# whwh747/A-Low-Texture-Robust-Hybrid-Feature-Based-Visual-Odometry

Measured on AMD Instinct MI355X. Metric: RGB-D frames/sec (640×480, 1k ORB + LSD + PEAC) at 1/2/4/8 GPUs, higher is better.
Workload: dtype u8/u16 integer + f32/f64; 1 GPU; 640x480 synthetic RGB-D, 1000 ORB (quota; 3/4 std + 1/4 lowtex scenes) + LSD lines + PEAC planes, 8192 frames per GPU per step (std640); frames_per_gpu=8192, parallelism=frames sharded, 1 rank(s), no data-path collective, distinct_frames=256, resident_bytes_per_frame_estimate=21100000

## Files before the change

a-low-texture-robust-hybrid-feature-based-visual-odometry_amd/csrc/peac.hip:

```cpp
#include <type_traits>
#include "hvo_internal.hpp"
#include <math.h>
#include <stdlib.h>
#include <string.h>
#include <vector>
#include <algorithm>

#define WIN 10
#define MIN_SUPPORT 3000
#define MAX_PLANES 64
#define SEG_D 16
#define SEG_I 8
#define LCAP 1024

struct PeacPlan {
    int w = 0, h = 0, pitch = 0, Nw = 0, Nh = 0, nblk = 0, segcap = 0, poolcap = 0, qcap = 0, batch = 0;
    uint16_t *d_depth = nullptr;
    double *d_segD = nullptr; int *d_segI = nullptr; int *d_pool = nullptr, *d_pool2 = nullptr;
    int *d_parent = nullptr, *d_dsize = nullptr, *d_eflag = nullptr;
    int *d_meta = nullptr;
    int *d_extracted = nullptr;
    int *d_blkmap = nullptr; int8_t *d_labels = nullptr; uint32_t *d_state = nullptr;
    int *d_queue = nullptr; int *d_plidmap = nullptr; int *d_isvalid = nullptr;
    hvo_plane *d_planes = nullptr;
    unsigned long long *d_adj = nullptr;
    void *d_hot = nullptr;
    double *d_hkey = nullptr, *d_m1k = nullptr; int *d_hid = nullptr;
    int *d_lq = nullptr;
    double c15 = 0, c60 = 0, c30 = 0;
    double ang_factor = 0, ang_near = 0;
    struct { Knob edges, gl, perm, lend, slots, heads_maxn, heads, heads_big, poolcap, ldsq, flood_t, flood_epl, flood_perm, flood_delay; } kn;
};

static PeacPlan *plan_of(hvo_ctx *ctx) { return (PeacPlan *)ctx->peac; }

static __device__ __forceinline__ void eig33_smallest_dev(double a, double b, double c, double d, double e, double f, double &l0, double v[3])
{
    const double tol = 2.220446049250313e-16 * (a + b + c);
    double l = 0.0;
    bool go = true;
#pragma unroll 1
    for (int it = 0; it < 8; it++) {
        if (!__any(go)) break;
        const double A = a - l, B = b - l, C = c - l;
        const double m1 = B * C - e * e, m2 = A * C - f * f, m3 = A * B - d * d;
        const double det = A * m1 - d * (d * C - e * f) + f * (d * e - B * f);
        const double dq = m1 + m2 + m3;
        const double q2 = -2.0 * (A + B + C);
        double disc = 4.0 * dq * dq + 6.0 * det * q2;
        if (disc < 0.0) disc = 0.0;
        const double ln = l + 3.0 * det / (dq + sqrt(disc));
        const bool adv = go && (dq > 0.0) && (ln > l);
        const double step = ln - l;
        if (adv) l = ln;
        go = adv && !(step <= tol);
    }
    const double A = a - l, B = b - l, C = c - l;
    const double m1 = B * C - e * e, m2 = A * C - f * f, m3 = A * B - d * d;
    const double am1 = fabs(m1), am2 = fabs(m2), am3 = fabs(m3);
    double x, y, z;
    if (am1 >= am2 && am1 >= am3) { x = m1; y = e * f - d * C; z = d * e - B * f; }
    else if (am2 >= am3) { x = e * f - d * C; y = m2; z = d * f - A * e; }
    else { x = d * e - B * f; y = d * f - A * e; z = m3; }
    const double n2 = x * x + y * y + z * z;
// ... 1154 lines not shown
            }
        }
        blkmap[b] = plid;
    }
    __syncthreads();
    const int tw = FS_TW(w), nrows = tw * FS_TH(h) * 4;
    for (int i = slice * 256 + tid; i < nrows; i += 256 * nslices) {
        const int t = i >> 2, ty = t / tw, tx = t - ty * tw;
        const int x0 = tx * 8, y = ty * 4 + (i & 3);
        if (y >= h) continue;
        const int by = y / WIN, bx0 = x0 / WIN, xs = (bx0 + 1) * WIN;
        const int l0 = (by < Nh && bx0 < Nw) ? blkmap[by * Nw + bx0] : -1, l1 = (by < Nh && bx0 + 1 < Nw) ? blkmap[by * Nw + bx0 + 1] : -1;
        unsigned dd[4];
        if (x0 + 8 <= pitch) { const uint4 q = *reinterpret_cast<const uint4 *>(D + (size_t)y * pitch + x0); dd[0] = q.x; dd[1] = q.y; dd[2] = q.z; dd[3] = q.w; }
        else { for (int k = 0; k < 4; k++) { const int xa = x0 + 2 * k; dd[k] = (xa < w ? (unsigned)D[(size_t)y * pitch + xa] : 0u) | ((xa + 1 < w ? (unsigned)D[(size_t)y * pitch + xa + 1] : 0u) << 16); } }
        unsigned st[8];
#pragma unroll
        for (int k = 0; k < 8; k++) {
            const int lab = x0 + k < xs ? l0 : l1;
            st[k] = FS_MAKE(lab, lab >= 0, (dd[k >> 1] >> (16 * (k & 1))) & 0xFFFFu);
        }
        uint4 *dst = reinterpret_cast<uint4 *>(state + (size_t)i * 8);
        dst[0] = make_uint4(st[0], st[1], st[2], st[3]); dst[1] = make_uint4(st[4], st[5], st[6], st[7]);
    }
}

struct RfArgs {
    ClArgs c;
    const uint16_t *depth; size_t dframe; int pitch, w, h;
    float fx, fy, cx, cy, dfac;
    int *blkmap; int *isvalid; uint32_t *state; int *queue; int qcap; int *plidmap; const int *perm;
    hvo_plane *planes; double c30;
    int flood_delay;
};

#ifndef FLOOD_HS_MUL
#define FLOOD_HS_MUL 1
#endif
#define FQ_PACK(x, y, pl) (((pl) << 26) | ((y) << 13) | (x))
static __device__ __forceinline__ void lds_barrier()
{
    __builtin_amdgcn_fence(__ATOMIC_RELEASE, "workgroup", "local");
    __builtin_amdgcn_s_barrier();
    __builtin_amdgcn_fence(__ATOMIC_ACQUIRE, "workgroup", "local");
}
template <int FLOOD_T, int EPL>
#ifdef HVO_WPE_FLOOD
__attribute__((amdgpu_waves_per_eu(HVO_WPE_FLOOD)))
#endif
__global__ __launch_bounds__(FLOOD_T) void k_peac_flood(RfArgs r, unsigned long long *__restrict__ adj_out)
{
    constexpr int NENT = FLOOD_T * EPL, NEV = NENT * 4;
    constexpr int FLOOD_HS = NEV * FLOOD_HS_MUL, FLOOD_HL = 4, FLOOD_NP = 4 * EPL;
    constexpr int NW = FLOOD_T / 64;
    static_assert(NEV <= 2048, "the group lists hold 11-bit event indices");
    constexpr int IXB = NEV > 1024 ? 11 : 10;
    constexpr unsigned IXM = (1u << IXB) - 1u;
    constexpr bool HL8 = NEV <= 256;
    typedef typename std::conditional<HL8, unsigned char, typename std::conditional<(NEV > 1024), unsigned int, unsigned short>::type>::type hl_t;
    __shared__ double pl[MAX_PLANES][7];
    __shared__ unsigned long long adj[MAX_PLANES], simok[MAX_PLANES];
    __shared__ int hkeys[FLOOD_HS], hcnt[FLOOD_HS];
    __shared__ __attribute__((aligned(16))) hl_t hlist[FLOOD_HS * FLOOD_HL];
    __shared__ uint2 rec[NEV];
    static_assert(FLOOD_HS >= NEV, "a ranked round indexes hkeys / hcnt by compact event index");
    __shared__ int wsum[EPL * NW], psum[FLOOD_NP * NW];
    __shared__ int s_nq, s_cx[2];
    const ClArgs &a = r.c;
    const int frame = r.perm ? r.perm[blockIdx.x] : (int)blockIdx.x, tid = threadIdx.x, lane = tid & 63, wv = tid >> 6;
    const int w = r.w, h = r.h, Nw = a.Nw, nblk = a.nblk;
    int *meta = a.meta + (size_t)frame * 16;
    const int nold = meta[2];
    const int *ext = a.extracted + (size_t)frame * 2 * MAX_PLANES;
    const double *segD = a.segD + (size_t)frame * a.segcap * SEG_D;
    const int *blkmap = r.blkmap + (size_t)frame * nblk;
    uint32_t *state = r.state + (size_t)frame * FS_FRAME(w, h);
    const int stw = FS_TW(w);
    int *queue = r.queue + (size_t)frame * r.qcap;
    int flags = 0;
    if (tid < MAX_PLANES) {
        adj[tid] = 0;
        if (tid < nold) { const double *sd = segD + (size_t)ext[tid] * SEG_D; for (int k = 0; k < 7; k++) pl[tid][k] = sd[9 + k]; }
    }
    for (int i = tid; i < FLOOD_HS; i += FLOOD_T) { hkeys[i] = -1; hcnt[i] = 0; }
    if (tid < 2) s_cx[tid] = 0;
    __syncthreads();
    if (tid < MAX_PLANES) {
        unsigned long long m = 0;
        if (tid < nold) for (int q = 0; q < nold; q++) {
            const double *P = pl[tid], *Q = pl[q];
            if (fabs(P[3] * Q[3] + P[4] * Q[4] + P[5] * Q[5]) >= r.c30) m |= 1ull << q;
        }
        simok[tid] = m;
    }
    constexpr int SEED_MAXG = 256;
    __shared__ int gtot[NW > 1 ? SEED_MAXG : 1];
    auto seed_count = [&](int b, int &m, int &up, int &lf, int &i, int &j) {
        int cnt = 0; m = -2; up = -2; lf = -2; i = 0; j = 0;
        if (b < nblk) {
            i = b / Nw; j = b - i * Nw; m = blkmap[b];
            up = i > 0 ? blkmap[b - Nw] : -2; lf = j > 0 ? blkmap[b - 1] : -2;
            if (m < 0) { if (i > 0 && up >= 0) cnt += WIN - 1; if (j > 0 && lf >= 0) cnt += WIN - 1; }
            else { if (i > 0 && up != m) cnt += WIN - 1; if (j > 0 && lf != m) cnt += WIN - 1; }
        }
        return cnt;
    };
    auto seed_write = [&](int pos, int cnt, int m, int up, int lf, int i, int j) {
        if (cnt && pos + cnt <= r.qcap) {
            const int x0 = j * WIN, y0 = i * WIN;
            if (m < 0) {
                if (i > 0 && up >= 0) for (int k = 1; k < WIN; ++k) queue[pos++] = FQ_PACK(x0 + k, y0 - 1, up);
                if (j > 0 && lf >= 0) for (int k = 0; k < WIN - 1; ++k) queue[pos++] = FQ_PACK(x0 - 1, y0 + k, lf);
            } else {
                if (i > 0 && up != m) for (int k = 0; k < WIN - 1; ++k) queue[pos++] = FQ_PACK(x0 + k, y0, m);
                if (j > 0 && lf != m) for (int k = 1; k < WIN; ++k) queue[pos++] = FQ_PACK(x0, y0 + k, m);
            }
        }
    };
    const int ngrp = (nblk + 63) / 64;
    if (NW > 1 && ngrp <= SEED_MAXG) {
        for (int g = wv; g < ngrp; g += NW) {
            int m, up, lf, i, j;
            int incl = seed_count(g * 64 + lane, m, up, lf, i, j);
            for (int o = 1; o < 64; o <<= 1) { int t = __shfl_up(incl, o); if (lane >= o) incl += t; }
// ... 97 lines not shown
                    if (act) actm |= 1u << (e * 4 + j);
                    const unsigned long long bm = __ballot(act);
                    below[e] += __popcll(bm & ltm); etot[e] += __popcll(bm);
                }
            }
            if (NW > 1) {
                if (lane == 0) for (int e = 0; e < EPL; e++) wsum[e * NW + wv] = etot[e];
                lds_barrier();
#pragma unroll
                for (int e = 0; e < EPL; e++) {
                    off[e] = wtot;
                    for (int i = 0; i < NW; i++) { const int v = wsum[e * NW + i]; if (i < wv) off[e] += v; wtot += v; }
                }
            } else {
#pragma unroll
                for (int e = 0; e < EPL; e++) { off[e] = wtot; wtot += etot[e]; }
            }
#pragma unroll
            for (int e = 0; e < EPL; e++) {
                const int plid = (int)((unsigned)q[e] >> 26), sx = q[e] & 8191, sy = (q[e] >> 13) & 8191;
                const int px[4] = { sx - 1, sx + 1, sx, sx }, py[4] = { sy, sy, sy - 1, sy + 1 };
                int c = off[e] + below[e];
#pragma unroll
                for (int j = 0; j < 4; j++) if (actm & (1u << (e * 4 + j))) { rec[c] = make_uint2((unsigned)FQ_PACK(px[j], py[j], plid), st[e][j]); c++; }
            }
        }
        lds_barrier();
        const int na = __builtin_amdgcn_readfirstlane(wtot);
        const int npass = (na + FLOOD_T - 1) / FLOOD_T;
#ifdef HVO_PEAC_TIMING
        if (tid == 0) { atomicAdd(&g_peac_t[30], (unsigned long long)na); atomicAdd(&g_peac_t[31], (unsigned long long)npass); }
#endif
        FT(1)
        unsigned eq[FLOOD_NP], es[FLOOD_NP]; float ed[FLOOD_NP], ecd[FLOOD_NP]; bool eok[FLOOD_NP], ev[FLOOD_NP], push[FLOOD_NP]; int hs[FLOOD_NP], eix[FLOOD_NP];
#pragma unroll
        for (int p = 0; p < FLOOD_NP; p++) {
            ev[p] = false; push[p] = false; eq[p] = 0; es[p] = 0; ed[p] = 0; ecd[p] = -1; eok[p] = false; hs[p] = 0; eix[p] = 0;
            if (p < npass) {
                const int c = p * FLOOD_T + tid;
                ev[p] = c < na;
                if (ev[p]) {
                    const uint2 R = rec[c];
                    eq[p] = R.x; es[p] = R.y;
                    const int ep = (int)(R.x >> 26), ex_ = (int)(R.x & 8191u), ey = (int)((R.x >> 13) & 8191u);
                    eix[p] = FS_IDX(ex_, ey, stw);
                    geom(pl[ep], ex_, ey, (int)(R.y >> 16), FS_LABEL(R.y), ecd[p], eok[p], ed[p]);
                    int s = (int)(((unsigned)eix[p] * 2654435761u) >> 19) & (FLOOD_HS - 1);
                    for (;;) {
                        const int old = atomicCAS(&hkeys[s], -1, eix[p]);
                        if (old == -1 || old == eix[p]) break;
                        s = (s + 1) & (FLOOD_HS - 1);
                    }
                    const int pos = atomicAdd(&hcnt[s], 1);
                    if (pos < FLOOD_HL) hlist[s * FLOOD_HL + pos] = HL8 ? (hl_t)c : (hl_t)((ep << IXB) | c);
                    hs[p] = s;
                }
            }
        }
        lds_barrier();
        bool first[FLOOD_NP], multi[FLOOD_NP]; int cnt[FLOOD_NP]; int cx = 0;
#pragma unroll
        for (int p = 0; p < FLOOD_NP; p++) {
            first[p] = false; multi[p] = false; cnt[p] = 1;
            if (p < npass && ev[p]) {
                cnt[p] = hcnt[hs[p]];
                first[p] = true;
                if (cnt[p] > FLOOD_HL) cx |= 2;
                else if (cnt[p] > 1) {
                    const unsigned me = ((eq[p] >> 26) << IXB) | (unsigned)(p * FLOOD_T + tid);
                    const hl_t *hp_ = &hlist[hs[p] * FLOOD_HL];
                    unsigned l[4] = { hp_[0], hp_[1], hp_[2], hp_[3] };
                    if (HL8) {
#pragma unroll
                        for (int t = 0; t < 4; t++) if (t < cnt[p]) l[t] |= (rec[l[t]].x >> 26) << IXB;
                    }
#pragma unroll
                    for (int t = 0; t < 4; t++) if (t < cnt[p]) {
                        if ((l[t] ^ me) >> IXB) multi[p] = true;
                        if ((l[t] & IXM) < (me & IXM)) first[p] = false;
                    }
                    if (multi[p]) cx |= FS_LABEL(es[p]) < 0 ? 1 : 2;
                }
            }
        }
        if (cx) atomicOr(&s_cx[par], cx);
        lds_barrier();
        const int cxr = s_cx[par];
        const bool complex_round = (cxr & 2) != 0;
        if (r.flood_delay && (cxr & 1) && wv == 0)
            for (int i = 0; i < r.flood_delay; i++) __builtin_amdgcn_s_sleep(127);
#pragma unroll
        for (int p = 0; p < FLOOD_NP; p++) if (p < npass && ev[p]) { hkeys[hs[p]] = -1; hcnt[hs[p]] = 0; }
        FT(2)
        int total = 0;
        if (!complex_round) {
#pragma unroll
            for (int p = 0; p < FLOOD_NP; p++) {
                if (p < npass && first[p] && !multi[p]) {
                    const int ep = (int)(eq[p] >> 26), trail = FS_LABEL(es[p]);
                    const bool closer = eok[p] && ecd[p] < ed[p];
                    if (eok[p] && trail >= 0 && ((simok[ep] >> trail) & 1ull)) { atomicOr(&adj[trail], 1ull << ep); atomicOr(&adj[ep], 1ull << trail); }
                    const int nl = closer ? ep : (trail < 0 ? max(trail - cnt[p], -6) : trail);
                    push[p] = closer;
                    if (nl != trail) state[eix[p]] = (es[p] & ~0xFFu) | ((unsigned)nl & 0xFFu);
                }
            }
            if (cxr & 1) {
                n_ranked++;
#ifdef HVO_PEAC_TIMING
                ft[6]++;
#endif
                if (NW > 1) lds_barrier();
#pragma unroll
                for (int p = 0; p < FLOOD_NP; p++) if (p < npass && multi[p]) hkeys[p * FLOOD_T + tid] = (int)(eok[p] ? __float_as_uint(ecd[p]) : 0xFFFFFFFFu);
                lds_barrier();
#pragma unroll
                for (int p = 0; p < FLOOD_NP; p++) {
                    if (p < npass && first[p] && multi[p]) {
                        const hl_t *hp_ = &hlist[hs[p] * FLOOD_HL];
                        unsigned l[4] = { hp_[0], hp_[1], hp_[2], hp_[3] };
                        if (HL8) {
#pragma unroll
                            for (int t = 0; t < 4; t++) if (t < cnt[p]) l[t] |= (rec[l[t]].x >> 26) << IXB;
                        }
                        int trail = FS_LABEL(es[p]); float dist = ed[p];
                        int last = -1;
                        for (int it = 0; it < cnt[p]; it++) {
                            unsigned best = 0; int c = 1 << 20;
#pragma unroll
                            for (int t = 0; t < 4; t++) { const int ct = (int)(l[t] & IXM); if (t < cnt[p] && ct > last && ct < c) { c = ct; best = l[t]; } }
                            const int ep = (int)(best >> IXB);
                            last = c;
                            const unsigned okcd = (unsigned)hkeys[c];
                            const bool ok = okcd != 0xFFFFFFFFu; const float cd = __uint_as_float(okcd);
                            const bool live = !(trail <= -6 || trail == ep);
                            const bool closer = live && ok && cd < dist;
                            if (live && ok && trail >= 0 && ((simok[ep] >> trail) & 1ull)) { atomicOr(&adj[trail], 1ull << ep); atomicOr(&adj[ep], 1ull << trail); }
                            trail = closer ? ep : ((live && trail < 0) ? trail - 1 : trail);
                            dist = closer ? cd : dist;
                            hcnt[c] = closer ? 1 : 0;
                        }
                        state[eix[p]] = (es[p] & ~0xFFu) | ((unsigned)trail & 0xFFu);
                    }
                }
                lds_barrier();
#pragma unroll
                for (int p = 0; p < FLOOD_NP; p++) if (p < npass && multi[p]) { push[p] = hcnt[p * FLOOD_T + tid] != 0; hkeys[p * FLOOD_T + tid] = -1; hcnt[p * FLOOD_T + tid] = 0; }
            }
            unsigned long long bm[FLOOD_NP]; int off[FLOOD_NP];
#pragma unroll
            for (int p = 0; p < FLOOD_NP; p++) { bm[p] = 0; if (p < npass) bm[p] = __ballot(push[p]); }
            if (NW > 1) {
                if (lane == 0) for (int p = 0; p < FLOOD_NP; p++) psum[p * NW + wv] = __popcll(bm[p]);
                lds_barrier();
#pragma unroll
                for (int p = 0; p < FLOOD_NP; p++) {
                    off[p] = total;
                    for (int i = 0; i < NW; i++) { const int v = psum[p * NW + i]; if (i < wv) off[p] += v; total += v; }
                }
            } else {
#pragma unroll
                for (int p = 0; p < FLOOD_NP; p++) { off[p] = total; total += __popcll(bm[p]); }
            }
#pragma unroll
            for (int p = 0; p < FLOOD_NP; p++) if (p < npass && push[p]) {
                const int pos = nq + off[p] + __popcll(bm[p] & ltm);
                if (pos < r.qcap) queue[pos] = (int)eq[p];
            }
        } else {
            n_serial++;
#ifdef HVO_PEAC_TIMING
            ft[5]++;
#endif
            if (tid == 0) {
                int nqs = nq;
                for (int e = 0; e < nent; e++) {
                    const int qq = queue[kq + e];
                    const int ep = (int)((unsigned)qq >> 26), x0 = qq & 8191, y0 = (qq >> 13) & 8191;
                    for (int j = 0; j < 4; j++) {
                        const int x = x0 + (j == 0 ? -1 : j == 1 ? 1 : 0), y = y0 + (j == 2 ? -1 : j == 3 ? 1 : 0);
                        if (x < 0 || x >= w || y < 0 || y >= h) continue;
                        const int ix = FS_IDX(x, y, stw);
                        const uint32_t s = state[ix];
                        int trail = FS_LABEL(s); float dist;
                        if ((s & FS_VALID) || trail <= -6 || trail == ep) continue;
                        float cd; bool ok;
                        geom(pl[ep], x, y, (int)(s >> 16), trail, cd, ok, dist);
                        if (ok) {
                            if (trail >= 0 && ((simok[ep] >> trail) & 1ull)) { atomicOr(&adj[trail], 1ull << ep); atomicOr(&adj[ep], 1ull << trail); }
                            if (cd < dist) { trail = ep; dist = cd; if (nqs < r.qcap) queue[nqs] = FQ_PACK(x, y, ep); nqs++; }
                            else if (trail < 0) trail -= 1;
                        } else if (trail < 0) trail -= 1;
                        state[ix] = (s & ~0xFFu) | ((unsigned)trail & 0xFFu);
                    }
                }
                s_nq = nqs - nq;
            }
            lds_barrier();
            total = s_nq;
        }
        nq += total;
        if (nq > r.qcap) { nq = r.qcap; flags |= 32; }
        kq += nent;
        par ^= 1;
        __syncthreads();
        FT(3)
    }
#ifdef HVO_PEAC_TIMING
    if (tid == 0) { for (int q = 0; q < 6; q++) atomicAdd(&g_peac_t[16 + q], ft[q]); for (int q = 6; q < 12; q++) atomicAdd(&g_peac_t[18 + q], ft[q]); atomicAdd(&g_peac_t[22], (unsigned long long)nq); atomicAdd(&g_peac_t[23], 1ull); }
#endif
    if (tid < MAX_PLANES) adj_out[(size_t)frame * MAX_PLANES + tid] = adj[tid];
    if (tid == 0) { meta[5] = nq; meta[7] = flags; meta[8] = n_rounds; meta[9] = n_ranked; meta[10] = n_serial; }
}

__global__ __launch_bounds__(64) void k_peac_final(RfArgs r, const unsigned long long *__restrict__ adj_in)
{
    __shared__ double hkey[MAX_PLANES]; __shared__ int hid[MAX_PLANES];
    __shared__ int lA[LCAP], lB[LCAP]; __shared__ double cm[64]; __shared__ int cN[64];
    const ClArgs &a = r.c;
    const int frame = blockIdx.x, lane = threadIdx.x;
    const int nblk = a.nblk;
    int *meta = a.meta + (size_t)frame * 16;
    const int nold = meta[2];
    int *ext = a.extracted + (size_t)frame * 2 * MAX_PLANES;
    double *segD = a.segD + (size_t)frame * a.segcap * SEG_D;
    int *segI = a.segI + (size_t)frame * a.segcap * SEG_I;
    int *pool = a.pool + (size_t)frame * a.poolcap, *pool2 = a.pool2 + (size_t)frame * a.poolcap;
    if (meta[6]) { int *t = pool; pool = pool2; pool2 = t; }
    const int *isvalid = r.isvalid + (size_t)frame * MAX_PLANES;
    int *plidmap = r.plidmap + (size_t)frame * MAX_PLANES;
    const unsigned long long *adj = adj_in + (size_t)frame * MAX_PLANES;
    int flags = meta[3] | meta[7];
    Heap H; H.key = hkey; H.id = hid; H.n = 0;
    int nseg = meta[0], pooltop = meta[1];
    if (pooltop + nold * MAX_PLANES > a.poolcap - 2 * a.nblk) pool_gc(segI, nseg, pool, pool2, pooltop);
    if (lane == 0) {
        for (int p = 0; p < nold; p++) {
            int *si = segI + (size_t)ext[p] * SEG_I;
            si[3] = pooltop + p * MAX_PLANES; si[4] = 0; si[5] = MAX_PLANES;
        }
        for (int p = 0; p < nold; p++) {
            int ids[MAX_PLANES], n = 0;
            for (int q = 0; q < nold; q++) if ((adj[p] >> q) & 1ull) ids[n++] = ext[q];
            for (int x = 1; x < n; x++) { int v = ids[x], y = x - 1; while (y >= 0 && ids[y] > v) { ids[y + 1] = ids[y]; y--; } ids[y + 1] = v; }
// ... 55 lines not shown
        }
    }
}

void peac_free(hvo_ctx *ctx)
{
    PeacPlan *P = plan_of(ctx);
    if (!P) return;
    void *ptrs[] = { P->d_depth, P->d_segD, P->d_segI, P->d_pool, P->d_pool2, P->d_parent, P->d_dsize, P->d_eflag, P->d_meta, P->d_extracted,
                     P->d_blkmap, P->d_labels, P->d_state, P->d_queue, P->d_plidmap, P->d_isvalid, P->d_planes, P->d_adj, P->d_hkey, P->d_m1k, P->d_hid, P->d_hot, P->d_lq };
    for (void *q : ptrs) if (q) (void)hipFree(q);
    delete P;
    ctx->peac = nullptr;
}

static int peac_build_plan(hvo_ctx *ctx, int w, int h, int batch);
static int peac_ensure_plan(hvo_ctx *ctx, int w, int h, int batch)
{
    PeacPlan *P = plan_of(ctx);
    if (P && P->w == w && P->h == h && P->batch >= batch) return HVO_OK;
    if (w < 2 * WIN || h < 2 * WIN || w > 4096 || h > 4096) return HVO_ERR_UNSUPPORTED;
    peac_free(ctx);
    const int rc = peac_build_plan(ctx, w, h, batch);
    if (rc) peac_free(ctx);
    return rc;
}

static int peac_build_plan(hvo_ctx *ctx, int w, int h, int batch)
{
    PeacPlan *P = new PeacPlan();
    ctx->peac = P;
    P->kn.edges.read("HVO_PEAC_EDGES"); P->kn.gl.read("HVO_PEAC_GL"); P->kn.perm.read("HVO_PEAC_PERM"); P->kn.lend.read("HVO_PEAC_LEND"); P->kn.slots.read("HVO_PEAC_SLOTS"); P->kn.heads_maxn.read("HVO_PEAC_HEADS_MAXN");
    P->kn.heads.read("HVO_PEAC_HEADS"); P->kn.heads_big.read("HVO_PEAC_HEADS_BIG"); P->kn.poolcap.read("HVO_PEAC_POOLCAP"); P->kn.ldsq.read("HVO_PEAC_LDSQ");
    P->kn.flood_t.read("HVO_FLOOD_T"); P->kn.flood_epl.read("HVO_FLOOD_EPL"); P->kn.flood_perm.read("HVO_FLOOD_PERM"); P->kn.flood_delay.read("HVO_FLOOD_DELAY");
    P->w = w; P->h = h; P->pitch = (w + 31) & ~31; P->Nw = w / WIN; P->Nh = h / WIN; P->nblk = P->Nw * P->Nh;
    P->segcap = 2 * P->nblk + 2 * MAX_PLANES; P->poolcap = 16 * P->nblk + 2 * MAX_PLANES * MAX_PLANES; P->qcap = 2 * w * h + 65536; P->batch = batch;
#define HVO_DEG2RAD(d) ((d) * 3.14159265358979323846 / 180.0)
    const double factor = (HVO_DEG2RAD(90.0) - HVO_DEG2RAD(15.0)) / (4000.0 - 500.0);
    P->c15 = cos(factor * 500.0 + HVO_DEG2RAD(15.0) - factor * 500.0);
    P->ang_factor = factor; P->ang_near = HVO_DEG2RAD(15.0);
    P->c60 = cos(HVO_DEG2RAD(60.0)); P->c30 = cos(HVO_DEG2RAD(30.0));
#undef HVO_DEG2RAD
    const size_t B = batch, npix = (size_t)w * h;
#define PA(ptr, n) HVO_HIP(hipMalloc((void **)&(ptr), (n)))
    PA(P->d_depth, B * P->pitch * (h + 1) * sizeof(uint16_t));
    PA(P->d_segD, B * P->segcap * SEG_D * sizeof(double));
    PA(P->d_segI, B * P->segcap * SEG_I * sizeof(int));
    PA(P->d_pool, B * P->poolcap * sizeof(int) + 64);
    PA(P->d_pool2, B * P->poolcap * sizeof(int) + 64);
    PA(P->d_parent, B * P->nblk * sizeof(int)); PA(P->d_dsize, B * P->nblk * sizeof(int)); PA(P->d_eflag, B * P->nblk * sizeof(int));
    PA(P->d_meta, B * 16 * sizeof(int)); PA(P->d_extracted, B * 2 * MAX_PLANES * sizeof(int));
    PA(P->d_blkmap, B * P->nblk * sizeof(int)); PA(P->d_labels, B * ((npix + 3) & ~(size_t)3)); PA(P->d_state, B * FS_FRAME(w, h) * sizeof(uint32_t));
    PA(P->d_queue, B * P->qcap * sizeof(int));
    PA(P->d_plidmap, B * MAX_PLANES * sizeof(int)); PA(P->d_isvalid, B * MAX_PLANES * sizeof(int));
    PA(P->d_planes, B * MAX_PLANES * sizeof(hvo_plane));
    PA(P->d_adj, B * MAX_PLANES * sizeof(unsigned long long));
    PA(P->d_hot, B * P->segcap * 128);
    { const size_t n0 = (P->segcap + 255) / 256; PA(P->d_hkey, B * n0 * 256 * sizeof(double)); PA(P->d_m1k, B * n0 * 16 * sizeof(double)); PA(P->d_hid, B * n0 * 16 * sizeof(int)); PA(P->d_lq, B * n0 * 256 * sizeof(int)); }
#undef PA
    HVO_HIP(hipMemsetAsync(P->d_depth, 0, B * P->pitch * (h + 1) * sizeof(uint16_t), ctx->s_peac));
    HVO_HIP(hipMemsetAsync(P->d_meta, 0, B * 16 * sizeof(int), ctx->s_peac));
    HVO_HIP(hipDeviceSynchronize());
    return HVO_OK;
}

bool peac_plan_covers(const hvo_ctx *ctx, int w, int h, int batch)
{
// ... 113 lines not shown
                a.tq_lds_keys = 1; lds = full;
                if (hvo_ensure_dyn_lds(reinterpret_cast<const void *>(k_peac_cluster<64, false>), lds)) return HVO_ERR_HIP;
            }
            hipLaunchKernelGGL((k_peac_cluster<64, false>), dim3(n), dim3(64), lds, st, a, n);
        }
        else if (use == 32) hipLaunchKernelGGL((k_peac_cluster<32, false>), dim3((n + 1) / 2), dim3(64), 2 * lq, st, a, n);
        else if (use == 16 && P->kn.poolcap.set && P->kn.poolcap.v >= 7 * a.nblk && P->kn.poolcap.v < a.poolcap) {
            ClArgs b = a; b.poolcap = P->kn.poolcap.v;
            if (!P->kn.slots.off() && !P->kn.lend.off() && slots_fit && P->d_lq) hipLaunchKernelGGL(k_peac_cluster_slots, dim3((n + 3) / 4), dim3(64), 4 * lq, st, b, n);
            else if (P->kn.lend.off()) hipLaunchKernelGGL((k_peac_cluster<16, false>), dim3((n + 3) / 4), dim3(64), 4 * lq, st, b, n);
            else hipLaunchKernelGGL((k_peac_cluster<16, true>), dim3((n + 3) / 4), dim3(64), 4 * lq, st, b, n);
        }
        else if (!P->kn.slots.off() && !P->kn.lend.off() && slots_fit && P->d_lq) hipLaunchKernelGGL(k_peac_cluster_slots, dim3((n + 3) / 4), dim3(64), 4 * lq, st, a, n);
        else if (P->kn.lend.off()) hipLaunchKernelGGL((k_peac_cluster<16, false>), dim3((n + 3) / 4), dim3(64), 4 * lq, st, a, n);
        else hipLaunchKernelGGL((k_peac_cluster<16, true>), dim3((n + 3) / 4), dim3(64), 4 * lq, st, a, n);
    }
    hvo_prof_end(ctx, id);
    id = hvo_prof_begin(ctx, "peac_refine", st);
    hipLaunchKernelGGL(k_peac_blkmap, dim3(n, n <= 64 ? 32 : n <= 1024 ? 4 : 1), dim3(256), 0, st, P->d_parent, P->d_dsize, P->d_segI, P->d_extracted, P->d_meta, P->d_blkmap,
                       P->d_isvalid, P->d_state, P->d_depth, dframe, P->pitch, P->nblk, P->Nw, P->Nh, P->w, P->h, P->segcap);
    RfArgs r;
    r.c = a; r.depth = P->d_depth; r.dframe = dframe; r.pitch = P->pitch; r.w = P->w; r.h = P->h;
    r.fx = p.fx; r.fy = p.fy; r.cx = p.cx; r.cy = p.cy; r.dfac = p.depth_map_factor;
    r.blkmap = P->d_blkmap; r.isvalid = P->d_isvalid; r.state = P->d_state; r.queue = P->d_queue; r.perm = nullptr;
    r.qcap = P->qcap; r.plidmap = P->d_plidmap; r.planes = P->d_planes; r.c30 = P->c30;
    r.flood_delay = std::min(std::max(P->kn.flood_delay.or_(0), 0), 64);
    {
        const int flood_t = P->kn.flood_t.or_(-1);
        const int ft = flood_t > 0 ? flood_t : (n >= 6144 ? 64 : n <= 8 ? 512 : 256);
        const int fe = P->kn.flood_epl.or_(1);
        r.perm = hvo_frame_perm(ctx, n);
        if ((ctx->sched == 5 || ctx->sched == 7) && ctx->fast_recorded && !ctx->serialize) HVO_HIP(hipStreamWaitEvent(st, ctx->ev_fast, 0));
        if (P->kn.flood_perm.off()) r.perm = nullptr;
        if (ft == 64 && fe == 2) hipLaunchKernelGGL((k_peac_flood<64, 2>), dim3(n), dim3(64), 0, st, r, P->d_adj);
        else if (ft == 64) hipLaunchKernelGGL((k_peac_flood<64, 1>), dim3(n), dim3(64), 0, st, r, P->d_adj);
        else if (ft == 512) hipLaunchKernelGGL((k_peac_flood<512, 1>), dim3(n), dim3(512), 0, st, r, P->d_adj);
        else if (ft == 256) hipLaunchKernelGGL((k_peac_flood<256, 1>), dim3(n), dim3(256), 0, st, r, P->d_adj);
        else hipLaunchKernelGGL((k_peac_flood<128, 1>), dim3(n), dim3(128), 0, st, r, P->d_adj);
    }
    hipLaunchKernelGGL(k_peac_final, dim3(n), dim3(64), 0, st, r, P->d_adj);
    hipLaunchKernelGGL(k_peac_relabel, dim3(64, n), dim3(256), 0, st, P->d_state, P->d_labels, P->d_plidmap, P->w, P->h, ((size_t)P->w * P->h + 3) & ~(size_t)3);
    hvo_prof_end(ctx, id);
    HVO_HIP(hipGetLastError());
    return HVO_OK;
}

int peac_download(hvo_ctx *ctx, int n, hvo_frame_out *out)
{
    const hipStream_t cs = hvo_copy_stream(ctx, ctx->s_peac);
    PeacPlan *P = plan_of(ctx);
    if (!P) return HVO_ERR_INVALID_ARG;
    std::vector<int> meta((size_t)n * 16);
    HVO_HIP(hipMemcpyAsync(meta.data(), P->d_meta, meta.size() * sizeof(int), hipMemcpyDeviceToHost, cs));
    HVO_HIP(hipStreamSynchronize(cs));
    const size_t npix = (size_t)P->w * P->h;
    std::vector<void *> dl(n, nullptr), dl8(n, nullptr), dp(n, nullptr); std::vector<size_t> bl(n, 0), bl8(n, 0), bp(n, 0);
    bool any32 = false, any8 = false;
    for (int f = 0; f < n; f++) { any32 |= out[f].labels != nullptr; any8 |= out[f].labels8 != nullptr; }
    for (int f = 0; f < n; f++) {
        const int nfin = meta[(size_t)f * 16 + 4], flags = meta[(size_t)f * 16 + 3];
        if (flags) out[f].status = HVO_ERR_CAPACITY;
        if (out[f].labels) { dl[f] = out[f].labels; bl[f] = npix; }
        if (out[f].labels8) { dl8[f] = out[f].labels8; bl8[f] = npix; }
        int m = nfin;
        if (out[f].planes) {
            if (m > out[f].pl_cap) { m = out[f].pl_cap; out[f].status = HVO_ERR_CAPACITY; }
            if (m > 0) { dp[f] = out[f].planes; bp[f] = (size_t)m * sizeof(hvo_plane); }
        }
        out[f].n_planes = m;
    }
    int rc = HVO_OK;
// ... 48 lines not shown
```

Baseline: 53750 frames/s.

## Split PEAC flood into slim few-plane kernel plus full kernel, pack per-event state

```diff
diff --git a/a-low-texture-robust-hybrid-feature-based-visual-odometry_amd/csrc/peac.hip b/a-low-texture-robust-hybrid-feature-based-visual-odometry_amd/csrc/peac.hip
--- a/a-low-texture-robust-hybrid-feature-based-visual-odometry_amd/csrc/peac.hip
+++ b/a-low-texture-robust-hybrid-feature-based-visual-odometry_amd/csrc/peac.hip
@@ -29,7 +29,7 @@
     int *d_lq = nullptr;
     double c15 = 0, c60 = 0, c30 = 0;
     double ang_factor = 0, ang_near = 0;
-    struct { Knob edges, gl, perm, lend, slots, heads_maxn, heads, heads_big, poolcap, ldsq, flood_t, flood_epl, flood_perm, flood_delay; } kn;
+    struct { Knob edges, gl, perm, lend, slots, heads_maxn, heads, heads_big, poolcap, ldsq, flood_t, flood_epl, flood_perm, flood_delay, flood_slim; } kn;
 };
 
 static PeacPlan *plan_of(hvo_ctx *ctx) { return (PeacPlan *)ctx->peac; }
@@ -1250,6 +1250,7 @@
     int *blkmap; int *isvalid; uint32_t *state; int *queue; int qcap; int *plidmap; const int *perm;
     hvo_plane *planes; double c30;
     int flood_delay;
+    int flood_lo;
 };
 
 #ifndef FLOOD_HS_MUL
@@ -1262,9 +1263,14 @@
     __builtin_amdgcn_s_barrier();
     __builtin_amdgcn_fence(__ATOMIC_ACQUIRE, "workgroup", "local");
 }
-template <int FLOOD_T, int EPL>
+#ifndef HVO_FLOOD_SLIM_WPE
+#define HVO_FLOOD_SLIM_WPE 6
+#endif
+template <int FLOOD_T, int EPL, int PMAX>
 #ifdef HVO_WPE_FLOOD
 __attribute__((amdgpu_waves_per_eu(HVO_WPE_FLOOD)))
+#else
+__attribute__((amdgpu_waves_per_eu(PMAX < MAX_PLANES ? HVO_FLOOD_SLIM_WPE : 1)))
 #endif
 __global__ __launch_bounds__(FLOOD_T) void k_peac_flood(RfArgs r, unsigned long long *__restrict__ adj_out)
 {
@@ -1276,8 +1282,10 @@
     constexpr unsigned IXM = (1u << IXB) - 1u;
     constexpr bool HL8 = NEV <= 256;
     typedef typename std::conditional<HL8, unsigned char, typename std::conditional<(NEV > 1024), unsigned int, unsigned short>::type>::type hl_t;
-    __shared__ double pl[MAX_PLANES][7];
-    __shared__ unsigned long long adj[MAX_PLANES], simok[MAX_PLANES];
+    static_assert(PMAX == 16 || PMAX == MAX_PLANES, "plane table sizes");
+    typedef typename std::conditional<(PMAX <= 32), unsigned, unsigned long long>::type pm_t;
+    __shared__ double pl[PMAX][7];
+    __shared__ pm_t adj[PMAX], simok[PMAX];
     __shared__ int hkeys[FLOOD_HS], hcnt[FLOOD_HS];
     __shared__ __attribute__((aligned(16))) hl_t hlist[FLOOD_HS * FLOOD_HL];
     __shared__ uint2 rec[NEV];
@@ -1289,6 +1297,7 @@
     const int w = r.w, h = r.h, Nw = a.Nw, nblk = a.nblk;
     int *meta = a.meta + (size_t)frame * 16;
     const int nold = meta[2];
+    if (nold > PMAX || nold <= r.flood_lo) return;
     const int *ext = a.extracted + (size_t)frame * 2 * MAX_PLANES;
     const double *segD = a.segD + (size_t)frame * a.segcap * SEG_D;
     const int *blkmap = r.blkmap + (size_t)frame * nblk;
@@ -1296,18 +1305,18 @@
     const int stw = FS_TW(w);
     int *queue = r.queue + (size_t)frame * r.qcap;
     int flags = 0;
-    if (tid < MAX_PLANES) {
+    if (tid < PMAX) {
         adj[tid] = 0;
         if (tid < nold) { const double *sd = segD + (size_t)ext[tid] * SEG_D; for (int k = 0; k < 7; k++) pl[tid][k] = sd[9 + k]; }
     }
     for (int i = tid; i < FLOOD_HS; i += FLOOD_T) { hkeys[i] = -1; hcnt[i] = 0; }
     if (tid < 2) s_cx[tid] = 0;
     __syncthreads();
-    if (tid < MAX_PLANES) {
-        unsigned long long m = 0;
+    if (tid < PMAX) {
+        pm_t m = 0;
         if (tid < nold) for (int q = 0; q < nold; q++) {
             const double *P = pl[tid], *Q = pl[q];
-            if (fabs(P[3] * Q[3] + P[4] * Q[4] + P[5] * Q[5]) >= r.c30) m |= 1ull << q;
+            if (fabs(P[3] * Q[3] + P[4] * Q[4] + P[5] * Q[5]) >= r.c30) m |= (pm_t)1 << q;
         }
         simok[tid] = m;
     }
@@ -1471,55 +1480,55 @@
         if (tid == 0) { atomicAdd(&g_peac_t[30], (unsigned long long)na); atomicAdd(&g_peac_t[31], (unsigned long long)npass); }
 #endif
         FT(1)
-        unsigned eq[FLOOD_NP], es[FLOOD_NP]; float ed[FLOOD_NP], ecd[FLOOD_NP]; bool eok[FLOOD_NP], ev[FLOOD_NP], push[FLOOD_NP]; int hs[FLOOD_NP], eix[FLOOD_NP];
+        constexpr unsigned W_EV = 1u << 16, W_OK = 1u << 17, W_FIRST = 1u << 18, W_MULTI = 1u << 19, W_PUSH = 1u << 20, W_CLOSER = 1u << 21;
+        static_assert(FLOOD_HS <= 4096 && FLOOD_HL < 8, "pass word: 12 bits of hash slot, 3 of group size");
+        unsigned pw[FLOOD_NP];
 #pragma unroll
         for (int p = 0; p < FLOOD_NP; p++) {
-            ev[p] = false; push[p] = false; eq[p] = 0; es[p] = 0; ed[p] = 0; ecd[p] = -1; eok[p] = false; hs[p] = 0; eix[p] = 0;
-            if (p < npass) {
-                const int c = p * FLOOD_T + tid;
-                ev[p] = c < na;
-                if (ev[p]) {
+            pw[p] = 0;
+            const int c = p * FLOOD_T + tid;
+            if (p < npass && c < na) {
+                const uint2 R = rec[c];
+                const int ep = (int)(R.x >> 26), ex_ = (int)(R.x & 8191u), ey = (int)((R.x >> 13) & 8191u);
+                const int eix = FS_IDX(ex_, ey, stw);
+                float cd, od; bool ok;
+                geom(pl[ep], ex_, ey, (int)(R.y >> 16), FS_LABEL(R.y), cd, ok, od);
+                int s = (int)(((unsigned)eix * 2654435761u) >> 19) & (FLOOD_HS - 1);
+                for (;;) {
+                    const int old = atomicCAS(&hkeys[s], -1, eix);
+                    if (old == -1 || old == eix) break;
+                    s = (s + 1) & (FLOOD_HS - 1);
+                }
+                const int pos = atomicAdd(&hcnt[s], 1);
+                if (pos < FLOOD_HL) hlist[s * FLOOD_HL + pos] = HL8 ? (hl_t)c : (hl_t)((ep << IXB) | c);
+                pw[p] = W_EV | (ok ? W_OK : 0u) | (ok && cd < od ? W_CLOSER : 0u) | (unsigned)s;
+            }
+        }
+        lds_barrier();
+        int cx = 0;
+#pragma unroll
+        for (int p = 0; p < FLOOD_NP; p++) {
+            if (p < npass && (pw[p] & W_EV)) {
+                const int c = p * FLOOD_T + tid, cnt = hcnt[pw[p] & 4095u];
+                bool first = true, multi = false;
+                if (cnt > FLOOD_HL) cx |= 2;
+                else if (cnt > 1) {
                     const uint2 R = rec[c];
-                    eq[p] = R.x; es[p] = R.y;
-                    const int ep = (int)(R.x >> 26), ex_ = (int)(R.x & 8191u), ey = (int)((R.x >> 13) & 8191u);
-                    eix[p] = FS_IDX(ex_, ey, stw);
-                    geom(pl[ep], ex_, ey, (int)(R.y >> 16), FS_LABEL(R.y), ecd[p], eok[p], ed[p]);
-                    int s = (int)(((unsigned)eix[p] * 2654435761u) >> 19) & (FLOOD_HS - 1);
-                    for (;;) {
-                        const int old = atomicCAS(&hkeys[s], -1, eix[p]);
-                        if (old == -1 || old == eix[p]) break;
-                        s = (s + 1) & (FLOOD_HS - 1);
-                    }
-                    const int pos = atomicAdd(&hcnt[s], 1);
-                    if (pos < FLOOD_HL) hlist[s * FLOOD_HL + pos] = HL8 ? (hl_t)c : (hl_t)((ep << IXB) | c);
-                    hs[p] = s;
-                }
-            }
-        }
-        lds_barrier();
-        bool first[FLOOD_NP], multi[FLOOD_NP]; int cnt[FLOOD_NP]; int cx = 0;
-#pragma unroll
-        for (int p = 0; p < FLOOD_NP; p++) {
-            first[p] = false; multi[p] = false; cnt[p] = 1;
-            if (p < npass && ev[p]) {
-                cnt[p] = hcnt[hs[p]];
-                first[p] = true;
-                if (cnt[p] > FLOOD_HL) cx |= 2;
-                else if (cnt[p] > 1) {
-                    const unsigned me = ((eq[p] >> 26) << IXB) | (unsigned)(p * FLOOD_T + tid);
-                    const hl_t *hp_ = &hlist[hs[p] * FLOOD_HL];
+                    const unsigned me = ((R.x >> 26) << IXB) | (unsigned)c;
+                    const hl_t *hp_ = &hlist[(pw[p] & 4095u) * FLOOD_HL];
                     unsigned l[4] = { hp_[0], hp_[1], hp_[2], hp_[3] };
                     if (HL8) {
 #pragma unroll
-                        for (int t = 0; t < 4; t++) if (t < cnt[p]) l[t] |= (rec[l[t]].x >> 26) << IXB;
+                        for (int t = 0; t < 4; t++) if (t < cnt) l[t] |= (rec[l[t]].x >> 26) << IXB;
                     }
 #pragma unroll
-                    for (int t = 0; t < 4; t++) if (t < cnt[p]) {
-                        if ((l[t] ^ me) >> IXB) multi[p] = true;
-                        if ((l[t] & IXM) < (me & IXM)) first[p] = false;
+                    for (int t = 0; t < 4; t++) if (t < cnt) {
+                        if ((l[t] ^ me) >> IXB) multi = true;
+                        if ((l[t] & IXM) < (me & IXM)) first = false;
                     }
-                    if (multi[p]) cx |= FS_LABEL(es[p]) < 0 ? 1 : 2;
+                    if (multi) cx |= FS_LABEL(R.y) < 0 ? 1 : 2;
                 }
+                pw[p] |= ((unsigned)min(cnt, 7) << 12) | (first ? W_FIRST : 0u) | (multi ? W_MULTI : 0u);
             }
         }
         if (cx) atomicOr(&s_cx[par], cx);
@@ -1529,19 +1538,20 @@
         if (r.flood_delay && (cxr & 1) && wv == 0)
             for (int i = 0; i < r.flood_delay; i++) __builtin_amdgcn_s_sleep(127);
 #pragma unroll
-        for (int p = 0; p < FLOOD_NP; p++) if (p < npass && ev[p]) { hkeys[hs[p]] = -1; hcnt[hs[p]] = 0; }
+        for (int p = 0; p < FLOOD_NP; p++) if (p < npass && (pw[p] & W_EV)) { hkeys[pw[p] & 4095u] = -1; hcnt[pw[p] & 4095u] = 0; }
         FT(2)
         int total = 0;
         if (!complex_round) {
 #pragma unroll
             for (int p = 0; p < FLOOD_NP; p++) {
-                if (p < npass && first[p] && !multi[p]) {
-                    const int ep = (int)(eq[p] >> 26), trail = FS_LABEL(es[p]);
-                    const bool closer = eok[p] && ecd[p] < ed[p];
-                    if (eok[p] && trail >= 0 && ((simok[ep] >> trail) & 1ull)) { atomicOr(&adj[trail], 1ull << ep); atomicOr(&adj[ep], 1ull << trail); }
-                    const int nl = closer ? ep : (trail < 0 ? max(trail - cnt[p], -6) : trail);
-                    push[p] = closer;
-                    if (nl != trail) state[eix[p]] = (es[p] & ~0xFFu) | ((unsigned)nl & 0xFFu);
+                if (p < npass && (pw[p] & (W_FIRST | W_MULTI)) == W_FIRST) {
+                    const uint2 R = rec[p * FLOOD_T + tid];
+                    const int ep = (int)(R.x >> 26), trail = FS_LABEL(R.y), cnt = (int)((pw[p] >> 12) & 7u);
+                    const bool ok = (pw[p] & W_OK) != 0, closer = (pw[p] & W_CLOSER) != 0;
+                    if (ok && trail >= 0 && ((simok[ep] >> trail) & 1u)) { atomicOr(&adj[trail], (pm_t)1 << ep); atomicOr(&adj[ep], (pm_t)1 << trail); }
+                    const int nl = closer ? ep : (trail < 0 ? max(trail - cnt, -6) : trail);
+                    if (closer) pw[p] |= W_PUSH;
+                    if (nl != trail) state[FS_IDX((int)(R.x & 8191u), (int)((R.x >> 13) & 8191u), stw)] = (R.y & ~0xFFu) | ((unsigned)nl & 0xFFu);
                 }
             }
             if (cxr & 1) {
@@ -1551,44 +1561,53 @@
 #endif
                 if (NW > 1) lds_barrier();
 #pragma unroll
-                for (int p = 0; p < FLOOD_NP; p++) if (p < npass && multi[p]) hkeys[p * FLOOD_T + tid] = (int)(eok[p] ? __float_as_uint(ecd[p]) : 0xFFFFFFFFu);
+                for (int p = 0; p < FLOOD_NP; p++) if (p < npass && (pw[p] & W_MULTI)) {
+                    const uint2 R = rec[p * FLOOD_T + tid];
+                    float cd, od; bool ok;
+                    geom(pl[R.x >> 26], (int)(R.x & 8191u), (int)((R.x >> 13) & 8191u), (int)(R.y >> 16), FS_LABEL(R.y), cd, ok, od);
+                    hkeys[p * FLOOD_T + tid] = (int)(ok ? __float_as_uint(cd) : 0xFFFFFFFFu);
+                }
                 lds_barrier();
 #pragma unroll
                 for (int p = 0; p < FLOOD_NP; p++) {
-                    if (p < npass && first[p] && multi[p]) {
-                        const hl_t *hp_ = &hlist[hs[p] * FLOOD_HL];
+                    if (p < npass && (pw[p] & (W_FIRST | W_MULTI)) == (W_FIRST | W_MULTI)) {
+                        const int cnt = (int)((pw[p] >> 12) & 7u);
+                        const hl_t *hp_ = &hlist[(pw[p] & 4095u) * FLOOD_HL];
                         unsigned l[4] = { hp_[0], hp_[1], hp_[2], hp_[3] };
                         if (HL8) {
 #pragma unroll
-                            for (int t = 0; t < 4; t++) if (t < cnt[p]) l[t] |= (rec[l[t]].x >> 26) << IXB;
+                            for (int t = 0; t < 4; t++) if (t < cnt) l[t] |= (rec[l[t]].x >> 26) << IXB;
                         }
-                        int trail = FS_LABEL(es[p]); float dist = ed[p];
+                        const uint2 R = rec[p * FLOOD_T + tid];
+                        float dist, cd0; bool ok0;
+                        geom(pl[R.x >> 26], (int)(R.x & 8191u), (int)((R.x >> 13) & 8191u), (int)(R.y >> 16), FS_LABEL(R.y), cd0, ok0, dist);
+                        int trail = FS_LABEL(R.y);
                         int last = -1;
-                        for (int it = 0; it < cnt[p]; it++) {
+                        for (int it = 0; it < cnt; it++) {
                             unsigned best = 0; int c = 1 << 20;
 #pragma unroll
-                            for (int t = 0; t < 4; t++) { const int ct = (int)(l[t] & IXM); if (t < cnt[p] && ct > last && ct < c) { c = ct; best = l[t]; } }
+                            for (int t = 0; t < 4; t++) { const int ct = (int)(l[t] & IXM); if (t < cnt && ct > last && ct < c) { c = ct; best = l[t]; } }
                             const int ep = (int)(best >> IXB);
                             last = c;
                             const unsigned okcd = (unsigned)hkeys[c];
                             const bool ok = okcd != 0xFFFFFFFFu; const float cd = __uint_as_float(okcd);
                             const bool live = !(trail <= -6 || trail == ep);
                             const bool closer = live && ok && cd < dist;
-                            if (live && ok && trail >= 0 && ((simok[ep] >> trail) & 1ull)) { atomicOr(&adj[trail], 1ull << ep); atomicOr(&adj[ep], 1ull << trail); }
+                            if (live && ok && trail >= 0 && ((simok[ep] >> trail) & 1u)) { atomicOr(&adj[trail], (pm_t)1 << ep); atomicOr(&adj[ep], (pm_t)1 << trail); }
                             trail = closer ? ep : ((live && trail < 0) ? trail - 1 : trail);
                             dist = closer ? cd : dist;
                             hcnt[c] = closer ? 1 : 0;
                         }
-                        state[eix[p]] = (es[p] & ~0xFFu) | ((unsigned)trail & 0xFFu);
+                        state[FS_IDX((int)(R.x & 8191u), (int)((R.x >> 13) & 8191u), stw)] = (R.y & ~0xFFu) | ((unsigned)trail & 0xFFu);
                     }
                 }
                 lds_barrier();
 #pragma unroll
-                for (int p = 0; p < FLOOD_NP; p++) if (p < npass && multi[p]) { push[p] = hcnt[p * FLOOD_T + tid] != 0; hkeys[p * FLOOD_T + tid] = -1; hcnt[p * FLOOD_T + tid] = 0; }
+                for (int p = 0; p < FLOOD_NP; p++) if (p < npass && (pw[p] & W_MULTI)) { if (hcnt[p * FLOOD_T + tid] != 0) pw[p] |= W_PUSH; hkeys[p * FLOOD_T + tid] = -1; hcnt[p * FLOOD_T + tid] = 0; }
             }
             unsigned long long bm[FLOOD_NP]; int off[FLOOD_NP];
 #pragma unroll
-            for (int p = 0; p < FLOOD_NP; p++) { bm[p] = 0; if (p < npass) bm[p] = __ballot(push[p]); }
+            for (int p = 0; p < FLOOD_NP; p++) { bm[p] = 0; if (p < npass) bm[p] = __ballot((pw[p] & W_PUSH) != 0); }
             if (NW > 1) {
                 if (lane == 0) for (int p = 0; p < FLOOD_NP; p++) psum[p * NW + wv] = __popcll(bm[p]);
                 lds_barrier();
@@ -1602,9 +1621,9 @@
                 for (int p = 0; p < FLOOD_NP; p++) { off[p] = total; total += __popcll(bm[p]); }
             }
 #pragma unroll
-            for (int p = 0; p < FLOOD_NP; p++) if (p < npass && push[p]) {
+            for (int p = 0; p < FLOOD_NP; p++) if (p < npass && (pw[p] & W_PUSH)) {
                 const int pos = nq + off[p] + __popcll(bm[p] & ltm);
-                if (pos < r.qcap) queue[pos] = (int)eq[p];
+                if (pos < r.qcap) queue[pos] = (int)rec[p * FLOOD_T + tid].x;
             }
         } else {
             n_serial++;
@@ -1626,7 +1645,7 @@
                         float cd; bool ok;
                         geom(pl[ep], x, y, (int)(s >> 16), trail, cd, ok, dist);
                         if (ok) {
-                            if (trail >= 0 && ((simok[ep] >> trail) & 1ull)) { atomicOr(&adj[trail], 1ull << ep); atomicOr(&adj[ep], 1ull << trail); }
+                            if (trail >= 0 && ((simok[ep] >> trail) & 1u)) { atomicOr(&adj[trail], (pm_t)1 << ep); atomicOr(&adj[ep], (pm_t)1 << trail); }
                             if (cd < dist) { trail = ep; dist = cd; if (nqs < r.qcap) queue[nqs] = FQ_PACK(x, y, ep); nqs++; }
                             else if (trail < 0) trail -= 1;
                         } else if (trail < 0) trail -= 1;
@@ -1648,7 +1667,7 @@
 #ifdef HVO_PEAC_TIMING
     if (tid == 0) { for (int q = 0; q < 6; q++) atomicAdd(&g_peac_t[16 + q], ft[q]); for (int q = 6; q < 12; q++) atomicAdd(&g_peac_t[18 + q], ft[q]); atomicAdd(&g_peac_t[22], (unsigned long long)nq); atomicAdd(&g_peac_t[23], 1ull); }
 #endif
-    if (tid < MAX_PLANES) adj_out[(size_t)frame * MAX_PLANES + tid] = adj[tid];
+    for (int i = tid; i < MAX_PLANES; i += FLOOD_T) adj_out[(size_t)frame * MAX_PLANES + i] = i < PMAX ? (unsigned long long)adj[i] : 0ull;
     if (tid == 0) { meta[5] = nq; meta[7] = flags; meta[8] = n_rounds; meta[9] = n_ranked; meta[10] = n_serial; }
 }
 
@@ -1770,7 +1789,7 @@
     ctx->peac = P;
     P->kn.edges.read("HVO_PEAC_EDGES"); P->kn.gl.read("HVO_PEAC_GL"); P->kn.perm.read("HVO_PEAC_PERM"); P->kn.lend.read("HVO_PEAC_LEND"); P->kn.slots.read("HVO_PEAC_SLOTS"); P->kn.heads_maxn.read("HVO_PEAC_HEADS_MAXN");
     P->kn.heads.read("HVO_PEAC_HEADS"); P->kn.heads_big.read("HVO_PEAC_HEADS_BIG"); P->kn.poolcap.read("HVO_PEAC_POOLCAP"); P->kn.ldsq.read("HVO_PEAC_LDSQ");
-    P->kn.flood_t.read("HVO_FLOOD_T"); P->kn.flood_epl.read("HVO_FLOOD_EPL"); P->kn.flood_perm.read("HVO_FLOOD_PERM"); P->kn.flood_delay.read("HVO_FLOOD_DELAY");
+    P->kn.flood_t.read("HVO_FLOOD_T"); P->kn.flood_epl.read("HVO_FLOOD_EPL"); P->kn.flood_perm.read("HVO_FLOOD_PERM"); P->kn.flood_delay.read("HVO_FLOOD_DELAY"); P->kn.flood_slim.read("HVO_FLOOD_SLIM");
     P->w = w; P->h = h; P->pitch = (w + 31) & ~31; P->Nw = w / WIN; P->Nh = h / WIN; P->nblk = P->Nw * P->Nh;
     P->segcap = 2 * P->nblk + 2 * MAX_PLANES; P->poolcap = 16 * P->nblk + 2 * MAX_PLANES * MAX_PLANES; P->qcap = 2 * w * h + 65536; P->batch = batch;
 #define HVO_DEG2RAD(d) ((d) * 3.14159265358979323846 / 180.0)
@@ -1950,11 +1969,16 @@
         r.perm = hvo_frame_perm(ctx, n);
         if ((ctx->sched == 5 || ctx->sched == 7) && ctx->fast_recorded && !ctx->serialize) HVO_HIP(hipStreamWaitEvent(st, ctx->ev_fast, 0));
         if (P->kn.flood_perm.off()) r.perm = nullptr;
-        if (ft == 64 && fe == 2) hipLaunchKernelGGL((k_peac_flood<64, 2>), dim3(n), dim3(64), 0, st, r, P->d_adj);
-        else if (ft == 64) hipLaunchKernelGGL((k_peac_flood<64, 1>), dim3(n), dim3(64), 0, st, r, P->d_adj);
-        else if (ft == 512) hipLaunchKernelGGL((k_peac_flood<512, 1>), dim3(n), dim3(512), 0, st, r, P->d_adj);
-        else if (ft == 256) hipLaunchKernelGGL((k_peac_flood<256, 1>), dim3(n), dim3(256), 0, st, r, P->d_adj);
-        else hipLaunchKernelGGL((k_peac_flood<128, 1>), dim3(n), dim3(128), 0, st, r, P->d_adj);
+        r.flood_lo = -1;
+        if (ft == 64 && fe != 2 && !P->kn.flood_slim.off()) {
+            hipLaunchKernelGGL((k_peac_flood<64, 1, 16>), dim3(n), dim3(64), 0, st, r, P->d_adj);
+            r.flood_lo = 16;
+        }
+        if (ft == 64 && fe == 2) hipLaunchKernelGGL((k_peac_flood<64, 2, MAX_PLANES>), dim3(n), dim3(64), 0, st, r, P->d_adj);
+        else if (ft == 64) hipLaunchKernelGGL((k_peac_flood<64, 1, MAX_PLANES>), dim3(n), dim3(64), 0, st, r, P->d_adj);
+        else if (ft == 512) hipLaunchKernelGGL((k_peac_flood<512, 1, MAX_PLANES>), dim3(n), dim3(512), 0, st, r, P->d_adj);
+        else if (ft == 256) hipLaunchKernelGGL((k_peac_flood<256, 1, MAX_PLANES>), dim3(n), dim3(256), 0, st, r, P->d_adj);
+        else hipLaunchKernelGGL((k_peac_flood<128, 1, MAX_PLANES>), dim3(n), dim3(128), 0, st, r, P->d_adj);
     }
     hipLaunchKernelGGL(k_peac_final, dim3(n), dim3(64), 0, st, r, P->d_adj);
     hipLaunchKernelGGL(k_peac_relabel, dim3(64, n), dim3(256), 0, st, P->d_state, P->d_labels, P->d_plidmap, P->w, P->h, ((size_t)P->w * P->h + 3) & ~(size_t)3);
```

New measurement: 55690 frames/s (median of 6 runs). +3.6%, better.
